# abowman6/CBET_RayTracing_3D

Measured on AMD Instinct MI355X. Metric: ray-steps/sec, OMEGA 60-beam 256^3 sweep, higher is better.
Workload: dtype f64

## Files before the change

### cbet_raytracing_3d_amd/csrc/cbet_trace_diag.h

```cpp
#ifndef CBET_TRACE_DIAG_H_
#define CBET_TRACE_DIAG_H_

#include "cbet_trace_common.h"

namespace cbet {

#ifdef CBET_DIAG_CLOCKS
#define CBET_IF_CLOCKS(...) __VA_ARGS__
#else
#define CBET_IF_CLOCKS(...)
#endif
#ifdef CBET_DIAG_FACES
#define CBET_IF_FACES(...) __VA_ARGS__
#else
#define CBET_IF_FACES(...)
#endif
#ifdef CBET_DIAG_CHAIN
#define CBET_IF_CHAIN(...) __VA_ARGS__
#else
#define CBET_IF_CHAIN(...)
#endif

struct WaveDiag {
    typedef unsigned long long u64;
    static constexpr bool kCountsWaveSteps = (0 CBET_IF_CLOCKS(+1) CBET_IF_FACES(+1) CBET_IF_CHAIN(+1)) != 0;
    CBET_IF_CLOCKS(u64 wait = 0, arm = 0, n_arm = 0, ret = 0, n_ret = 0, t_start, t_wait, t_arm, t_ret;)
    CBET_IF_FACES(unsigned near_steps = 0, near_axes = 0, arm_steps = 0;)
    CBET_IF_CHAIN(u64 chain = 0, t_chain = 0;)

    static __device__ __forceinline__ void stamp(u64 &t) { asm volatile("s_memtime %0" : "=&s"(t) : : "memory"); }
    static __device__ __forceinline__ void stamp_wait(u64 &t) { asm volatile("s_memtime %0\n\ts_waitcnt lgkmcnt(0)" : "=&s"(t) : : "memory"); }
    static __device__ __forceinline__ u64 since(u64 t0)
    {
        u64 t1;
        asm volatile("s_memtime %0\n\ts_waitcnt lgkmcnt(0)" : "=&s"(t1) : "s"(t0) : "memory");
        return t1 - t0;
    }

    __device__ __forceinline__ void begin() { CBET_IF_CLOCKS(stamp_wait(t_start);) }
    __device__ __forceinline__ void step_begin(int near)
    {
        (void)near;
        CBET_IF_FACES(near_steps += near != 0 ? 1 : 0; near_axes += __builtin_popcount((unsigned)near);)
    }
    __device__ __forceinline__ void wait_begin() { CBET_IF_CLOCKS(stamp(t_wait);) }
    __device__ __forceinline__ void wait_end()
    {
        CBET_IF_CLOCKS(wait += since(t_wait);)
        CBET_IF_CHAIN(stamp_wait(t_chain);)
    }
    __device__ __forceinline__ void chain_end() { CBET_IF_CHAIN(chain += since(t_chain);) }
    __device__ __forceinline__ void arm_begin()
    {
        CBET_IF_FACES(arm_steps += 1;)
        CBET_IF_CLOCKS(stamp(t_arm);)
    }
    __device__ __forceinline__ void arm_end() { CBET_IF_CLOCKS(arm += since(t_arm); n_arm += 1;) }
    __device__ __forceinline__ void retire_begin() { CBET_IF_CLOCKS(stamp(t_ret);) }
    __device__ __forceinline__ void retire_end() { CBET_IF_CLOCKS(ret += since(t_ret); n_ret += 1;) }
    __device__ __forceinline__ bool report(const TraceArgs &a, int lane, int tot_steps, int tot_rays, unsigned wave_steps)
    {
        auto put = [&](int slot, u64 v) { atomicAdd(&a.counters[slot], v); };
        if (kCountsWaveSteps && lane == 0) {
            CBET_IF_CLOCKS(u64 t_end; stamp_wait(t_end);)
            put(kCntSteps, (u64)tot_steps);
            put(kCntWaveSteps, (u64)wave_steps);
#if defined(CBET_DIAG_CLOCKS)
            put(kCntGlobalAtomics, wait);
            put(kCntEvictions, arm);
            put(kCntWaveStepsWide, n_arm);
            put(kCntSlabsRetired, t_end - t_start);
            put(kCntRays, ret);
            put(kCntWaveStepsMiss, n_ret);
#elif defined(CBET_DIAG_CHAIN)
            put(kCntRays, (u64)tot_rays);
            put(kCntGlobalAtomics, chain);
#elif defined(CBET_DIAG_FACES)
            put(kCntRays, (u64)tot_rays);
            put(kCntWaveStepsWide, (u64)near_steps);
            put(kCntWaveStepsMiss, (u64)near_axes);
            put(kCntSlabsRetired, (u64)arm_steps);
#endif
        }
        (void)tot_rays;
        return kCountsWaveSteps;
    }
};
#undef CBET_IF_CLOCKS
#undef CBET_IF_FACES
#undef CBET_IF_CHAIN

}

#endif
```

### cbet_raytracing_3d_amd/csrc/cbet_trace_window.hip

```cpp
#include <hip/hip_runtime.h>

#include <cstddef>
#include <type_traits>

#if defined(__HIP_DEVICE_COMPILE__) && !defined(__gfx950__)
#error "cbet_trace_window.hip is written for gfx950 (CDNA4) only"
#endif

#include "cbet_trace_common.h"
#include "cbet_trace_diag.h"

namespace cbet {
namespace {

#define CBET_BALLOT(cond) __builtin_amdgcn_ballot_w64(cond)
#define CBET_LANES(mask) __builtin_amdgcn_inverse_ballot_w64(mask)

template <int WX_, int WY_, int WZ_, bool PAD, bool XORSW = false>
struct Tile {
    static constexpr int WX = WX_, WY = WY_, WZ = WZ_;
    static constexpr int XM = WX - 1, YM = WY - 1, ZM = WZ - 1;
    static constexpr bool ROT = PAD && WZ == 16;
    static constexpr int YS = (PAD && !ROT) ? WZ + 1 : WZ;
    static constexpr int XS = (PAD && !ROT) ? WY * YS + 4 : WY * WZ;
    static constexpr bool XOR = ROT && XORSW;
    static __device__ __forceinline__ int zr(int tx, int ty, int tz)
    {
        return XOR ? (tz ^ ((tx & 3) << 2) ^ (ty << 1)) : (ROT ? ((tz + 7 * tx + 3 * ty) & ZM) : tz);
    }
    static_assert(!XOR || (WX == 8 && WY == 8 && WZ == 16), "the swizzle terms are written for the 8 x 8 x 16 box");
    static __device__ __forceinline__ int xterm(int tx) { return __mul24(tx, XS * 8 + 32) & ~0x80; }
    static __device__ __forceinline__ int yterm(int ty) { return __mul24(ty, YS * 8 + 16); }
    static constexpr int N = WX * XS;
    static constexpr int SX = WX - 2, SY = WY - 2, SZ = WZ - 2;
    static constexpr bool BRICK = WZ == 16 && WY == 8;
    static constexpr int DT = WX * WY * WZ;
    static __device__ __forceinline__ int slot_d(int tx, int ty, int tz) { return (tx * WY + ty) * WZ + tz; }
};

struct Origin {
    int x, y, z;
};

template <int M>
__device__ __forceinline__ int abs_in(int o, int r) { return o + ((r - o) & M); }

template <int C>
struct Corner {
    static constexpr int index = C;
    template <class V> static __device__ __forceinline__ V x(V v0, V v1) { return (C & 1) ? v1 : v0; }
    template <class V> static __device__ __forceinline__ V z(V v0, V v1) { return (C & 2) ? v1 : v0; }
    template <class V> static __device__ __forceinline__ V y(V v0, V v1) { return (C & 4) ? v1 : v0; }
};
template <class F>
__device__ __forceinline__ void each_corner(F f)
{
    f(Corner<0>{}); f(Corner<1>{}); f(Corner<2>{}); f(Corner<3>{}); f(Corner<4>{}); f(Corner<5>{}); f(Corner<6>{}); f(Corner<7>{});
}

struct WaveCounters {
    int n_atomics = 0;
    int n_miss = 0;
    unsigned steps_miss = 0;
    unsigned slabs_bsteps = 0;
    int pend = 0;
    [[no_unique_address]] WaveDiag dg;
};

template <bool W32>
struct Grid {
    double *p;
};
template <bool W32>
__device__ __forceinline__ void grid_add(const TraceArgs &a, Grid<W32> g, int node, double v)
{
    if constexpr (W32) global_add(a, reinterpret_cast<double *>(reinterpret_cast<char *>(g.p) + ((unsigned)node * 8u)), v);
    else global_add(a, &g.p[node], v);
}
template <bool W32>
__device__ __forceinline__ void grid_add_far(const TraceArgs &a, Grid<W32> g, long index, double v) { global_add(a, &g.p[index], v); }

template <class G>
__device__ __forceinline__ void write_back(const TraceArgs &a, double *tile, int slot, G edep, int node, double v, WaveCounters &wc)
{
    wc.pend += (CBET_BALLOT(v != 0.0) != 0ull) ? 1 : 0;
    if (v != 0.0) {
        tile[slot] = 0.0;
        ++wc.n_atomics;
        grid_add(a, edep, node, v);
    }
}
template <class G>
__device__ __forceinline__ void write_back_far(const TraceArgs &a, double *tile, int slot, G edep, long index, double v, WaveCounters &wc)
{
    wc.pend += (CBET_BALLOT(v != 0.0) != 0ull) ? 1 : 0;
    if (v != 0.0) {
        grid_add_far(a, edep, index, v);
        tile[slot] = 0.0;
        ++wc.n_atomics;
    }
}

template <class F>
__device__ __forceinline__ void miss_add8(unsigned long long hbm_m, WaveCounters &wc, F add8)
{
    if (hbm_m != 0ull) {
        wc.pend += 8;
        if (CBET_LANES(hbm_m)) add8();
    }
}

template <class T, int AX, int COUNT, class G>
__device__ __forceinline__ void retire_planes(const TraceArgs &a, double *tile, const Origin &o, int coord, int step,
                                              int lane, G edep, int sXh, int sYh, WaveCounters &wc)
{
    constexpr int WO = AX == 0 ? T::WY : T::WX, OM = WO - 1;
    constexpr int IT = (WO * T::WZ + kWave - 1) / kWave;
    constexpr int RS = kWave / T::WZ;
    static_assert(IT == 1 || (IT == 2 && 2 * RS == WO), "a plane is one entry per lane, or two in the halves of the other axis");
    static_assert(!T::XOR || IT == 1 || (RS == 4 && T::YS == 16 && T::XS == 128), "the second entry's slot is written for the 8 x 8 x 16 box");
    constexpr int SLOT_X = AX == 0 ? (RS * T::YS) ^ ((2 * RS) & T::ZM) : RS * T::XS;
    const int r0 = lane / T::WZ, r1 = lane & T::ZM, k = abs_in<T::ZM>(o.z, r1);
    const int d0 = (r0 - (AX == 0 ? o.y : o.x)) & OM, dnode = ((d0 & RS) ? -RS : RS) * (AX == 0 ? sYh : sXh);
    const bool in_plane = !(WO * T::WZ < kWave) || lane < WO * T::WZ;
    double v[COUNT * IT];
    int slot[COUNT * IT], node[COUNT * IT];
#pragma unroll
    for (int pl = 0; pl < COUNT; ++pl) {
        const int c = coord + pl * step;
        const int fixed = c & (AX == 0 ? T::XM : T::YM);
#pragma unroll
        for (int e = 0; e < IT; ++e) {
            const int q = pl * IT + e, re = r0 + e * RS;
            if (e == 1 && T::XOR) {
                slot[q] = slot[q - 1] ^ SLOT_X;
                node[q] = node[q - 1] + dnode;
            } else if (AX == 0) {
                slot[q] = fixed * T::XS + re * T::YS + T::zr(fixed, re, r1);
                node[q] = c * sXh + __mul24(abs_in<T::YM>(o.y, re), sYh) + k;
            } else {
                slot[q] = re * T::XS + fixed * T::YS + T::zr(re, fixed, r1);
                node[q] = __mul24(abs_in<T::XM>(o.x, re), sXh) + c * sYh + k;
            }
            const bool ok = in_plane && CBET_AUDIT(a, (unsigned)slot[q] < (unsigned)T::N);
            v[q] = ok ? tile[slot[q]] : 0.0;
        }
    }
#pragma unroll
    for (int q = 0; q < COUNT * IT; ++q) write_back(a, tile, slot[q], edep, node[q], v[q], wc);
}

template <class T, int AX, int NC, class G>
__device__ __forceinline__ void retire_plane(const TraceArgs &a, double *tile, const Origin &o, int coord, int lane,
                                             G edep, int sXh, int sYh, WaveCounters &wc, int coff, long gstride)
{
    constexpr int WO = AX == 0 ? T::WY : T::WX;
    constexpr int IT = (WO * T::WZ + kWave - 1) / kWave;
    const int fixed = coord & (AX == 0 ? T::XM : T::YM);
#pragma unroll
    for (int e = 0; e < IT; ++e) {
        const int idx = e * kWave + lane;
        const bool in_plane = !(WO * T::WZ < kWave) || idx < WO * T::WZ;
        const int r0 = idx / T::WZ, r1 = idx & T::ZM;
        int slot, node, slot_d;
        const int k = abs_in<T::ZM>(o.z, r1);
        if (AX == 0) {
            slot = fixed * T::XS + r0 * T::YS + T::zr(fixed, r0, r1);
            slot_d = T::slot_d(fixed, r0, r1);
            node = coord * sXh + __mul24(abs_in<T::YM>(o.y, r0), sYh) + k;
        } else {
            slot = r0 * T::XS + fixed * T::YS + T::zr(r0, fixed, r1);
            slot_d = T::slot_d(r0, fixed, r1);
            node = __mul24(abs_in<T::XM>(o.x, r0), sXh) + coord * sYh + k;
        }
        const bool ok = in_plane && CBET_AUDIT(a, (unsigned)slot < (unsigned)T::N);
        const double v = ok ? tile[slot] : 0.0;
        if (NC > 1) {
#pragma unroll
            for (int q = 1; q < NC; ++q) {
                const int sq = coff + (q - 1) * T::DT + slot_d;
                write_back_far(a, tile, sq, edep, q * gstride + node, ok ? tile[sq] : 0.0, wc);
            }
        }
        write_back(a, tile, slot, edep, node, v, wc);
    }
}

template <class T, int NC, class G>
__device__ __forceinline__ void retire_zplane(const TraceArgs &a, double *tile, const Origin &o, int coord, int lane,
                                              G edep, int sXh, int sYh, WaveCounters &wc, int coff, long gstride)
{
    static_assert(T::WX * T::WY <= kWave, "one z-plane entry per lane");
    const int r0 = lane / T::WY, r1 = lane & T::YM, fixed = coord & T::ZM;
    const int slot = r0 * T::XS + r1 * T::YS + T::zr(r0, r1, fixed);
    const int node = __mul24(abs_in<T::XM>(o.x, r0), sXh) + __mul24(abs_in<T::YM>(o.y, r1), sYh) + coord;
    const bool ok = (!(T::WX * T::WY < kWave) || lane < T::WX * T::WY) && CBET_AUDIT(a, (unsigned)slot < (unsigned)T::N);
    const double v = ok ? tile[slot] : 0.0;
    if (NC > 1) {
        const int slot_d = T::slot_d(r0, r1, fixed);
#pragma unroll
        for (int q = 1; q < NC; ++q) {
            const int sq = coff + (q - 1) * T::DT + slot_d;
            write_back_far(a, tile, sq, edep, q * gstride + node, ok ? tile[sq] : 0.0, wc);
        }
    }
    write_back(a, tile, slot, edep, node, v, wc);
}

template <class T, class G>
__device__ __forceinline__ void retire_zbrick(const TraceArgs &a, double *tile, const Origin &o, int zb, int lane,
                                              G edep, int sXh, int sYh, WaveCounters &wc)
{
    static_assert(T::WY == 8 && T::WZ == 16, "a brick is 8 rows of 8 planes per tile x index");
    const int ty = lane >> 3, kz = lane & 7;
    const int tz = (zb + kz) & T::ZM;
    const int base_node = __mul24(abs_in<T::YM>(o.y, ty), sYh) + zb + kz;
    constexpr int ROUND = 4;
#pragma unroll
    for (int t0 = 0; t0 < T::WX; t0 += ROUND) {
        double v[ROUND];
        int slot[ROUND];
#pragma unroll
        for (int q = 0; q < ROUND; ++q) {
            slot[q] = (t0 + q) * T::XS + ty * T::YS + T::zr(t0 + q, ty, tz);
            v[q] = CBET_AUDIT(a, (unsigned)slot[q] < (unsigned)T::N) ? tile[slot[q]] : 0.0;
        }
#pragma unroll
        for (int q = 0; q < ROUND; ++q) write_back(a, tile, slot[q], edep, abs_in<T::XM>(o.x, t0 + q) * sXh + base_node, v[q], wc);
    }
}

template <class T, int NC, class G>
__device__ __forceinline__ void flush_box(const TraceArgs &a, double *tile, const Origin &o, int lane, G edep,
                                          int sXh, int sYh, WaveCounters &wc, int coff, long gstride)
{
    for (int t = 0; t < T::WX; ++t)
        retire_plane<T, 0, NC>(a, tile, o, o.x + t, lane, edep, sXh, sYh, wc, coff, gstride);
}

__device__ __forceinline__ int follow_plane_axis(int r, unsigned long long mm, int S)
{
    const unsigned long long edge = __builtin_amdgcn_ballot_w64((unsigned)(r - 1) >= (unsigned)(S - 1)) & mm;
    if (edge == 0ull) return 0;
    const unsigned long long hi = __builtin_amdgcn_ballot_w64(r >= S) & edge;
    const bool at_hi = hi != 0ull, at_lo = hi != edge;
    if (at_hi == at_lo) return 0;
    if (at_hi) {
        if ((__builtin_amdgcn_ballot_w64(r <= 1) & mm) != 0ull) return (__builtin_amdgcn_ballot_w64(r > S) & mm) != 0ull ? 1 : 0;
        return (S >= 6 && (__builtin_amdgcn_ballot_w64(r <= 2) & mm) == 0ull) ? 2 : 1;
    }
    if ((__builtin_amdgcn_ballot_w64(r >= S - 1) & mm) != 0ull) return (__builtin_amdgcn_ballot_w64(r < 0) & mm) != 0ull ? -1 : 0;
    return (S >= 6 && (__builtin_amdgcn_ballot_w64(r >= S - 2) & mm) == 0ull) ? -2 : -1;
}

__device__ __forceinline__ int follow_brick_axis(int r, unsigned long long mm)
{
    if ((__builtin_amdgcn_ballot_w64((unsigned)r > 14u) & mm) == 0ull) return 0;
    const bool below = (__builtin_amdgcn_ballot_w64(r < 0) & mm) != 0ull, above = (__builtin_amdgcn_ballot_w64(r > 14) & mm) != 0ull;
    const bool needs_lo = (__builtin_amdgcn_ballot_w64(r <= 7) & mm) != 0ull, needs_hi = (__builtin_amdgcn_ballot_w64(r >= 7) & mm) != 0ull;
    return (below && !needs_hi) ? -1 : ((above && !needs_lo) ? 1 : 0);
}

template <class T, int NC, class G>
__device__ __forceinline__ bool follow_box(const TraceArgs &a, double *tile, Origin &o, unsigned long long mm, int lx,
                                           int ly, int lz, int lane, G edep, int sXh, int sYh, WaveCounters &wc,
                                           int coff, long gstride)
{
    auto leave = [&](auto axis, int d, int lo, int hi) {
        constexpr int AX = decltype(axis)::value;
        const int first = d < 0 ? hi : lo, step = d < 0 ? -1 : 1, n = d < 0 ? -d : d;
        if constexpr (NC == 1) {
            if (n == 2) retire_planes<T, AX, 2>(a, tile, o, first, step, lane, edep, sXh, sYh, wc);
            else retire_planes<T, AX, 1>(a, tile, o, first, step, lane, edep, sXh, sYh, wc);
        } else {
            for (int q = 0; q < n; ++q) retire_plane<T, AX, NC>(a, tile, o, first + q * step, lane, edep, sXh, sYh, wc, coff, gstride);
        }
    };
    const int dx = follow_plane_axis(lx - o.x, mm, T::SX);
    const int dy = follow_plane_axis(ly - o.y, mm, T::SY);
    if (dx != 0) { wc.dg.retire_begin(); leave(std::integral_constant<int, 0>{}, dx, o.x, o.x + T::WX - 1); wc.dg.retire_end(); }
    o.x += dx;
    if (dy != 0) { wc.dg.retire_begin(); leave(std::integral_constant<int, 1>{}, dy, o.y, o.y + T::WY - 1); wc.dg.retire_end(); }
    o.y += dy;
    int dz;
    if constexpr (T::BRICK) {
        dz = 8 * follow_brick_axis(lz - o.z, mm);
        if (dz != 0) { wc.dg.retire_begin(); retire_zbrick<T>(a, tile, o, dz < 0 ? o.z + 8 : o.z, lane, edep, sXh, sYh, wc); wc.dg.retire_end(); }
    } else {
        dz = follow_plane_axis(lz - o.z, mm, T::SZ);
        if (dz != 0)
            retire_zplane<T, NC>(a, tile, o, dz < 0 ? o.z + T::WZ - 1 : o.z, lane, edep, sXh, sYh, wc, coff, gstride);
        for (int q = 1; q < (dz < 0 ? -dz : dz); ++q)
            retire_zplane<T, NC>(a, tile, o, dz < 0 ? o.z + T::WZ - 1 - q : o.z + q, lane, edep, sXh, sYh, wc, coff, gstride);
    }
    o.z += dz;
    const bool moved = (dx | dy | dz) != 0;
    wc.slabs_bsteps += moved ? (1u << 16) : 0u;
    return moved;
}

template <class T>
__device__ __forceinline__ bool holds(const Origin &o, int lx, int ly, int lz)
{
    return (unsigned)(lx - o.x) <= (unsigned)T::SX && (unsigned)(ly - o.y) <= (unsigned)T::SY &&
           (unsigned)(lz - o.z) <= (unsigned)T::SZ;
}

template <class T>
__device__ __forceinline__ int box_near_axes(const Origin &o, int nx, int ny, int nz)
{
    const int lo = kRelocateDeep + 1;
    const unsigned tx = (unsigned)((o.x - lo) | (nx - 3 - T::SX - o.x)), ty = (unsigned)((o.y - lo) | (ny - 3 - T::SY - o.y)),
                   tz = (unsigned)((o.z - lo) | (nz - 3 - T::SZ - o.z));
    return (int)((tx >> 31) | ((ty >> 31) << 1) | ((tz >> 31) << 2));
}

typedef double dbl2 __attribute__((ext_vector_type(2)));

template <bool WIDE>
__device__ __forceinline__ void record_issue(const StepRecord *base, unsigned cell, dbl2 &kxy, dbl2 &kzk)
{
    if constexpr (WIDE) {
        const char *p = reinterpret_cast<const char *>(base) + ((unsigned long long)cell << 5);
        asm volatile("global_load_dwordx4 %0, %2, off\n\tglobal_load_dwordx4 %1, %2, off offset:16\n\t; CBET_RECORD_ISSUE %0 %1"
                     : "=&v"(kxy), "=&v"(kzk)
                     : "v"(p)
                     : "memory");
    } else {
        const unsigned off = cell << 5;
        asm volatile("s_nop 4\n\tglobal_load_dwordx4 %0, %2, %3\n\tglobal_load_dwordx4 %1, %2, %3 offset:16\n\t; CBET_RECORD_ISSUE %0 %1"
                     : "=&v"(kxy), "=&v"(kzk)
                     : "v"(off), "s"(base)
                     : "memory");
    }
}

__device__ __forceinline__ void record_wait(dbl2 &kxy, dbl2 &kzk, int pend)
{
    asm volatile("; CBET_RECORD_WAIT %0 %1\n\t"
                 "s_cmp_eq_u32 %2, 0\n\t"
                 "s_cbranch_scc1 .Lrw_0_%=\n\t"
                 "s_cmp_ge_u32 %2, 8\n\t"
                 "s_cbranch_scc1 .Lrw_8_%=\n\t"
                 "s_cmp_ge_u32 %2, 4\n\t"
                 "s_cbranch_scc1 .Lrw_4_%=\n\t"
                 "s_cmp_ge_u32 %2, 2\n\t"
                 "s_cbranch_scc1 .Lrw_2_%=\n\t"
                 "s_waitcnt vmcnt(1)\n\t"
                 "s_branch .Lrw_end_%=\n"
                 ".Lrw_2_%=:\n\t"
                 "s_waitcnt vmcnt(2)\n\t"
                 "s_branch .Lrw_end_%=\n"
                 ".Lrw_4_%=:\n\t"
                 "s_waitcnt vmcnt(4)\n\t"
                 "s_branch .Lrw_end_%=\n"
                 ".Lrw_8_%=:\n\t"
                 "s_waitcnt vmcnt(8)\n\t"
                 "s_branch .Lrw_end_%=\n"
                 ".Lrw_0_%=:\n\t"
                 "s_waitcnt vmcnt(0)\n"
                 ".Lrw_end_%=:"
                 : "+v"(kxy), "+v"(kzk)
                 : "s"(pend)
                 : "memory", "scc");
}

__device__ __forceinline__ void record_wait_all(dbl2 &kxy, dbl2 &kzk)
{
    asm volatile("; CBET_RECORD_WAIT %0 %1\n\ts_waitcnt vmcnt(0)" : "+v"(kxy), "+v"(kzk) : : "memory");
}

__device__ __forceinline__ void exit_planes_load(dbl2 &bx, dbl2 &by, dbl2 &bz)
{
    const void *args = (const void *)__builtin_amdgcn_kernarg_segment_ptr();
    asm volatile("s_load_dwordx4 %0, %3, %4\n\ts_load_dwordx4 %1, %3, %5\n\ts_load_dwordx4 %2, %3, %6\n\ts_waitcnt lgkmcnt(0)"
                 : "=&s"(bx), "=&s"(by), "=&s"(bz)
                 : "s"(args), "i"(offsetof(TraceArgs, exit_planes)), "i"(offsetof(TraceArgs, exit_planes) + 16),
                   "i"(offsetof(TraceArgs, exit_planes) + 32));
}

__device__ __forceinline__ int add3(int a, int b, int c)
{
    int r;
    asm("v_add3_u32 %0, %1, %2, %3" : "=v"(r) : "v"(a), "v"(b), "v"(c));
    return r;
}

__device__ __forceinline__ int xad1(int f, int c)
{
    int r;
    asm("v_xad_u32 %0, %1, 1, %2" : "=v"(r) : "v"(f), "v"(c));
    return r;
}

__device__ __forceinline__ double max_abs3(double a, double b, double c)
{
    double r;
    asm("v_max_f64 %0, |%1|, |%2|" : "=v"(r) : "v"(a), "v"(b));
    asm("v_max_f64 %0, %1, |%2|" : "=v"(r) : "v"(r), "v"(c));
    return r;
}

__device__ __forceinline__ void commit(int &var, int value)
{
    asm volatile("s_mov_b32 %0, %1" : "+s"(var) : "s"(__builtin_amdgcn_readfirstlane(value)));
}
__device__ __forceinline__ void commit(unsigned long long &var, unsigned long long value)
{
    asm volatile("s_mov_b64 %0, %1" : "+s"(var) : "s"(value));
}
__device__ __forceinline__ void commit_v(int &var, int value) { asm volatile("v_mov_b32 %0, %1" : "+v"(var) : "v"(value)); }

__device__ __forceinline__ void cell_step(int &c, unsigned long long up, unsigned long long dn)
{
    asm("s_nop 1\n\tv_addc_co_u32_e64 %0, vcc, 0, %0, %1\n\tv_subbrev_co_u32_e64 %0, vcc, 0, %0, %2" : "+v"(c) : "s"(up), "s"(dn) : "vcc");
}
__device__ __forceinline__ void cell_step3(int &ci, int &cj, int &ck, unsigned long long upx, unsigned long long dnx,
                                           unsigned long long upy, unsigned long long dny, unsigned long long upz,
                                           unsigned long long dnz)
{
    asm("s_nop 1\n\t"
        "v_addc_co_u32_e64 %0, vcc, 0, %0, %3\n\tv_addc_co_u32_e64 %1, vcc, 0, %1, %5\n\tv_addc_co_u32_e64 %2, vcc, 0, %2, %7\n\t"
        "v_subbrev_co_u32_e64 %0, vcc, 0, %0, %4\n\tv_subbrev_co_u32_e64 %1, vcc, 0, %1, %6\n\tv_subbrev_co_u32_e64 %2, vcc, 0, %2, %8"
        : "+v"(ci), "+v"(cj), "+v"(ck)
        : "s"(upx), "s"(dnx), "s"(upy), "s"(dny), "s"(upz), "s"(dnz)
        : "vcc");
}

__device__ __forceinline__ int mad24(int a, int b, int c)
{
    int r;
    asm("s_nop 1\n\tv_mad_i32_i24 %0, %1, %2, %3" : "=v"(r) : "v"(a), "s"(b), "v"(c));
    return r;
}


#ifdef CBET_DEBUG_BOUNDS
constexpr bool kAudited = true;
#else
constexpr bool kAudited = false;
#endif
constexpr double kNearTol = 0.5001;
constexpr double kFarJump = 1.4998;

template <int WZ, bool GENERIC, int CBET, bool STATS>
__global__ void __launch_bounds__(kWave, (CBET == 4) ? 1 : 4) k_trace_window(const TraceArgs a)
{
    using T = Tile<8, 8, WZ, true, CBET == 0>;
    using TB = Tile<4, 8, 8, false>;
    constexpr bool IDX64 = GENERIC;
    constexpr int NC = (CBET == 4) ? 4 : 1;
    constexpr bool ACC = (CBET == 0);
    constexpr bool PIPE = ACC;
    constexpr int NSLOT = T::N + TB::N;
    constexpr int NLDS = NSLOT + (NC - 1) * T::DT;
    __shared__ double s_val[NLDS];
    const int lane = threadIdx.x;

    int beam, patch;
    if (!work_item(a, blockIdx.x, beam, patch)) return;
    const Grid<!IDX64> edep{a.edep + (long)(beam - a.grid_beam0) * a.grid_stride};
    const bool absorb = GENERIC ? (a.absorption == 1) : true;

    Ray s = {};
    int li;
    const bool launched = launch_lane(a, beam, patch, lane, s, li);
    unsigned long long live = __ballot(launched);
    if (live == 0ull) return;
    const int tot_rays = __popcll(live);

    const int nx = a.nx, ny = a.ny, nz = a.nz;
    const int sYh = a.sYh, sXh = a.sXh;
    unsigned cell = launched ? (unsigned)((s.ci * ny + s.cj) * nz + s.ck) : 0u;
    double fcx = (double)s.ci, fcy = (double)s.cj, fcz = (double)s.ck;
    int tot_steps = 0;
    WaveCounters wc;

    double *const tileA = s_val, *const tileB = s_val + T::N;
    Origin oA{0, 0, 0}, oB{0, 0, 0};
    unsigned long long hbm = 0ull;
    int b_active = 0;
    {
        const int src = ((live >> 27) & 1ull) ? 27 : (__ffsll((long long)live) - 1);
        for (int z = lane; z < NLDS; z += kWave) s_val[z] = 0.0;
        oA.x = __builtin_amdgcn_readlane(s.ci, src) + 1 - T::WX / 2;
        oA.y = __builtin_amdgcn_readlane(s.cj, src) + 1 - T::WY / 2;
        oA.z = __builtin_amdgcn_readlane(s.ck, src) + 1 - 4;
        if (T::BRICK) oA.z &= ~7;
        __syncthreads();
    }
    int near = 7;
    wc.dg.begin();

    dbl2 rec_kxy, rec_kzk;
    const StepRecord *rec_base = a.steprec;
    asm volatile("" : "+s"(rec_base));
    double dt = a.dt;
    auto gather_record = [&]() {
        unsigned c = CBET_LANES(live) ? cell : 0u;
        asm("" : "+v"(c));
#ifdef CBET_DEBUG_BOUNDS
        if (!(c < a.audit_nodes)) { audit_fail(a); c = 0u; }
#endif
        record_issue<IDX64>(rec_base, c, rec_kxy, rec_kzk);
        wc.pend = 0;
    };
    auto await_record = [&]() {
        wc.dg.wait_begin();
        if (CBET == 0 && !kAudited) record_wait(rec_kxy, rec_kzk, wc.pend);
        else record_wait_all(rec_kxy, rec_kzk);
        wc.dg.wait_end();
    };
    gather_record();
    await_record();
    const double *const gk = CBET && a.gain ? a.gain + (long)(beam - a.grid_beam0) * a.hsize : nullptr;
    double gained = 0.0;

    const bool flx = (lane & 1) != 0, fly = (lane & 2) != 0, flz = (lane & 8) != 0;
    const int pfx = flx ? 1 : 0, pfy = fly ? 1 : 0, pfz = flz ? 1 : 0;

    double q0 = 0.0, q1 = 0.0, q2 = 0.0, q3 = 0.0;

    int slow = 7;
    double Fx0 = 0, Fx1 = 0, Fy0 = 0, Fy1 = 0, Fz0 = 0, Fz1 = 0;
    int X0 = 0, X1 = 0, Y0 = 0, Y1 = 0, Z0 = 0, Z1 = 0;
    double inc = 0.0;
    int tile_off = 0;
    unsigned long long miss_m = 0ull;
    int own_slot = 0, own_node = 0;
    auto lds_add8 = [&](const double *w) {
        auto add = [&](int byte, double v) {
            if (CBET_AUDIT(a, (unsigned)byte < (unsigned)NSLOT * 8u))
                __hip_atomic_fetch_add(static_cast<double *>(__builtin_assume_aligned(reinterpret_cast<char *>(s_val) + byte, 8)),
                                       v, __ATOMIC_RELAXED, __HIP_MEMORY_SCOPE_WORKGROUP);
        };
        if constexpr (T::XOR) {
            int ax0, ax1, by0, by1, cz0, cz1;
            if (b_active == 0) {
                ax0 = T::xterm(X0 & T::XM); ax1 = T::xterm(X1 & T::XM);
                by0 = T::yterm(Y0 & T::YM); by1 = T::yterm(Y1 & T::YM);
                cz0 = (Z0 & T::ZM) << 3; cz1 = (Z1 & T::ZM) << 3;
            } else {
                const bool toB = tile_off != 0;
                const int xm = toB ? TB::XM : T::XM, zm = toB ? TB::ZM : T::ZM;
                const int xmul = toB ? TB::XS * 8 : T::XS * 8 + 32, ymul = toB ? TB::YS * 8 : T::YS * 8 + 16;
                const int keep = toB ? ~0 : ~0x80, off8 = tile_off * 8;
                static_assert(TB::YM == T::YM, "one y mask for both boxes");
                ax0 = (__mul24(X0 & xm, xmul) & keep) | off8; ax1 = (__mul24(X1 & xm, xmul) & keep) | off8;
                by0 = __mul24(Y0 & T::YM, ymul); by1 = __mul24(Y1 & T::YM, ymul);
                cz0 = (Z0 & zm) << 3; cz1 = (Z1 & zm) << 3;
            }
            auto at = [](int ax, int by, int cz) { return (int)__builtin_amdgcn_bitop3_b32(ax, by, cz, 0x96); };
            each_corner([=](auto c) { add(at(c.x(ax0, ax1), c.y(by0, by1), c.z(cz0, cz1)), w[c.index]); });
        } else {
            auto add8 = [&](int xm, int ym, int zm, int xs, int ys, int off, int rot) {
                const int xa = X0 & xm, xb = X1 & xm, ya = Y0 & ym, yb = Y1 & ym;
                const int x0 = __mul24(xa, xs * 8) + off * 8, x1 = __mul24(xb, xs * 8) + off * 8;
                const int y0 = __mul24(ya, ys * 8), y1 = __mul24(yb, ys * 8);
                const int ra = 7 * xa * rot, rb = 7 * xb * rot, sa = 3 * ya * rot, sb = 3 * yb * rot;
                auto zb = [&](int z, int r) { return ((z + r) & zm) * 8; };
                if constexpr (T::ROT) {
                    const int xy00 = x0 | y0, xy10 = x1 | y0, xy01 = x0 | y1, xy11 = x1 | y1, zm8 = zm * 8;
                    auto at = [&](int xy, int z, int r) { return (((z + r) * 8) & zm8) | xy; };
                    each_corner([&](auto c) {
                        add(at(c.y(c.x(xy00, xy10), c.x(xy01, xy11)), c.z(Z0, Z1), c.x(ra, rb) + c.y(sa, sb)), w[c.index]);
                    });
                } else {
                    each_corner([&](auto c) {
                        add(add3(c.x(x0, x1), c.y(y0, y1), zb(c.z(Z0, Z1), c.x(ra, rb) + c.y(sa, sb))), w[c.index]);
                    });
                }
            };
            if (b_active == 0) {
                add8(T::XM, T::YM, T::ZM, T::XS, T::YS, 0, T::ROT ? 1 : 0);
            } else {
                const bool toB = tile_off != 0;
                add8(toB ? TB::XM : T::XM, toB ? TB::YM : T::YM, toB ? TB::ZM : T::ZM, toB ? TB::XS : T::XS,
                     toB ? TB::YS : T::YS, tile_off, (T::ROT && !toB) ? 1 : 0);
            }
        }
    };
    auto hbm_add8 = [&](const double *w) {
        const int nX0 = __mul24(X0, sXh), nX1 = __mul24(X1, sXh), nY0 = __mul24(Y0, sYh), nY1 = __mul24(Y1, sYh);
        each_corner([&](auto c) { grid_add(a, edep, c.x(nX0, nX1) + c.y(nY0, nY1) + c.z(Z0, Z1), w[c.index]); });
        wc.n_atomics += 8;
    };

    auto deposit_step = [&](unsigned long long lds_m, unsigned long long hbm_m) {
        const double zi0 = Fz0 * inc, zi1 = Fz1 * inc;
        const double zy00 = zi0 * Fy0, zy10 = zi1 * Fy0, zy01 = zi0 * Fy1, zy11 = zi1 * Fy1;
        double wgt[8];
        wgt[0] = zy00 * Fx0;
        wgt[1] = zy00 * Fx1;
        wgt[2] = zy10 * Fx0;
        wgt[3] = zy10 * Fx1;
        wgt[4] = zy01 * Fx0;
        wgt[5] = zy01 * Fx1;
        wgt[6] = zy11 * Fx0;
        wgt[7] = zy11 * Fx1;
        if (CBET_LANES(lds_m)) lds_add8(wgt);
        miss_add8(hbm_m, wc, [&]() {
            hbm_add8(wgt);
            ++wc.n_miss;
        });
        if (CBET == 4) {
            const bool inbox = CBET_LANES(lds_m);
            if (inbox && tile_off == 0) {
                if (CBET_AUDIT(a, (unsigned)(own_slot + 2 * T::DT) < (unsigned)NLDS)) {
                    __hip_atomic_fetch_add(&s_val[own_slot], q1, __ATOMIC_RELAXED, __HIP_MEMORY_SCOPE_WORKGROUP);
                    __hip_atomic_fetch_add(&s_val[own_slot + T::DT], q2, __ATOMIC_RELAXED, __HIP_MEMORY_SCOPE_WORKGROUP);
                    __hip_atomic_fetch_add(&s_val[own_slot + 2 * T::DT], q3, __ATOMIC_RELAXED, __HIP_MEMORY_SCOPE_WORKGROUP);
                }
            } else if (inbox || CBET_LANES(hbm_m)) {
                grid_add_far(a, edep, a.comp_stride + own_node, q1);
                grid_add_far(a, edep, 2 * a.comp_stride + own_node, q2);
                grid_add_far(a, edep, 3 * a.comp_stride + own_node, q3);
                wc.n_atomics += 3;
            }
        }
    };

    double S[8] = {0, 0, 0, 0, 0, 0, 0, 0};
    unsigned long long restart_m = 0ull;
    bool p_odd = true;
    auto accumulate = [&]() {
        const double zi0 = Fz0 * inc, zi1 = Fz1 * inc;
        const double zy00 = zi0 * Fy0, zy10 = zi1 * Fy0, zy01 = zi0 * Fy1, zy11 = zi1 * Fy1;
        const double k = CBET_LANES(restart_m) ? 0.0 : 1.0;
        auto add = [&](double &sum, double w) { asm("v_fma_f64 %0, %0, %1, %2" : "+v"(sum) : "v"(k), "v"(w)); };
        add(S[0], zy00 * Fx0);
        add(S[1], zy00 * Fx1);
        add(S[2], zy10 * Fx0);
        add(S[3], zy10 * Fx1);
        add(S[4], zy01 * Fx0);
        add(S[5], zy01 * Fx1);
        add(S[6], zy11 * Fx0);
        add(S[7], zy11 * Fx1);
    };
    auto flush_sums = [&](unsigned long long lds_m, unsigned long long hbm_m) {
        if (CBET_LANES(lds_m)) lds_add8(S);
        miss_add8(hbm_m, wc, [&]() { hbm_add8(S); });
    };

    auto step_tail = [&](int &tt) {
    asm volatile("" : "+v"(Fx0), "+v"(Fx1), "+v"(Fy0), "+v"(Fy1), "+v"(Fz0), "+v"(Fz1));
    await_record();
    if (absorb) {
        inc = rec_kzk.y * s.uray;
        s.uray -= inc;
    } else {
        inc = s.uray;
    }
    if (CBET >= 2) inc = q0;
    if constexpr (ACC && !PIPE) accumulate();
    unsigned long long died = CBET_BALLOT(s.uray <= s.ustop);
    const int faces = slow | near;
    if (faces != 0) {
        dbl2 bx, by, bz;
        exit_planes_load(bx, by, bz);
        if (faces & 1) died |= CBET_BALLOT(s.px < bx.x) | CBET_BALLOT(s.px > bx.y);
        if (faces & 2) died |= CBET_BALLOT(s.py < by.x) | CBET_BALLOT(s.py > by.y);
        if (faces & 4) died |= CBET_BALLOT(s.pz < bz.x) | CBET_BALLOT(s.pz > bz.y);
    }
    died &= live;
    if (died != 0ull) {
        asm volatile("");
        commit(tot_steps, tot_steps + __popcll(died) * (tt + 1));
        if constexpr (PIPE) {
            accumulate();
            asm volatile("v_mov_b64 %0, 0" : "+v"(inc));
            commit(restart_m, 0ull);
        }
        if constexpr (ACC) flush_sums(died & ~miss_m, died & miss_m);
        else deposit_step(died & ~miss_m, died & miss_m);
        commit(live, live & ~died);
        commit(hbm, hbm & live);
        commit(miss_m, miss_m & live);
        if (live == 0ull) commit(tt, a.nt - 1);
    }
    __builtin_amdgcn_wave_barrier();
    };

    for (int tt = 0; tt < a.nt; ++tt) {
        if constexpr (STATS || WaveDiag::kCountsWaveSteps) wc.steps_miss += 1u << 16;
        wc.dg.step_begin(near);
        s.vx -= rec_kxy.x;
        s.vy -= rec_kxy.y;
        s.vz -= rec_kzk.x;
        asm volatile("" : "+s"(dt));
        s.px += s.vx * dt;
        s.py += s.vy * dt;
        s.pz += s.vz * dt;
        const double fx = (s.px - a.xmin) * a.inv_dx;
        const double fy = (s.py - a.ymin) * a.inv_dy;
        const double fz = (s.pz - a.zmin) * a.inv_dz;
        const double g0x = fx - fcx, g0y = fy - fcy, g0z = fz - fcz;
        const unsigned long long upx = CBET_BALLOT(g0x >= kNearTol), dnx = CBET_BALLOT(g0x < kNearTol - 1.0),
                                 upy = CBET_BALLOT(g0y >= kNearTol), dny = CBET_BALLOT(g0y < kNearTol - 1.0),
                                 upz = CBET_BALLOT(g0z >= kNearTol), dnz = CBET_BALLOT(g0z < kNearTol - 1.0);
        slow = ((CBET_BALLOT(!(max_abs3(g0x, g0y, g0z) < kFarJump)) & live) != 0ull) ? 7 : near;
        if (slow == 0) {
            cell_step3(s.ci, s.cj, s.ck, upx, dnx, upy, dny, upz, dnz);
        } else {
            if (slow & 1) s.ci = relocate_closed(s.ci, fx, nx);
            else cell_step(s.ci, upx, dnx);
            if (slow & 2) s.cj = relocate_closed(s.cj, fy, ny);
            else cell_step(s.cj, upy, dny);
            if (slow & 4) s.ck = relocate_closed(s.ck, fz, nz);
            else cell_step(s.ck, upz, dnz);
        }
        const unsigned new_cell = (unsigned)mad24(mad24(s.ci, ny, s.cj), nz, s.ck);
        unsigned long long moved_m = 0ull;
        if constexpr (ACC) moved_m = CBET_BALLOT(new_cell != cell);
        cell = new_cell;
        gather_record();
        wc.dg.chain_end();
        asm volatile("" : "+v"(s.ci), "+v"(s.cj), "+v"(s.ck), "+v"(inc));
        fcx = (double)s.ci;
        fcy = (double)s.cj;
        fcz = (double)s.ck;
        if constexpr (!ACC) deposit_step(live & ~miss_m, miss_m);
        if constexpr (PIPE) accumulate();
        const double ox = (fx - fcx) - 0.5, oy = (fy - fcy) - 0.5, oz = (fz - fcz) - 0.5;
        const bool ngx = ox < 0, ngy = oy < 0, ngz = oz < 0;
        const bool all_negative = (live & ~(CBET_BALLOT(ngx) & CBET_BALLOT(ngy) & CBET_BALLOT(ngz))) == 0ull;
        if constexpr (ACC) {
            const unsigned long long fl_m = (all_negative && !p_odd) ? (live & moved_m) : live;
            if (fl_m != 0ull) {
                if (miss_m == 0ull) flush_sums(fl_m, 0ull);
                else flush_sums(fl_m & ~miss_m, fl_m & miss_m);
            }
            restart_m = fl_m;
            p_odd = !all_negative;
        }
        factor_pair(ox, pfx, Fx0, Fx1);
        factor_pair(oy, pfy, Fy0, Fy1);
        factor_pair(oz, pfz, Fz0, Fz1);
        int rx, ry, rz;
        if (all_negative) {
            rx = s.ci - oA.x;
            ry = s.cj - oA.y;
            rz = s.ck - oA.z;
            asm("" : "+v"(rx), "+v"(ry), "+v"(rz));
            X0 = xad1(pfx, s.ci); X1 = s.ci + pfx;
            Y0 = xad1(pfy, s.cj); Y1 = s.cj + pfy;
            Z0 = xad1(pfz, s.ck); Z1 = s.ck + pfz;
        } else {
            const int lx = s.ci + 1 - (ngx ? 1 : 0);
            const int ly = s.cj + 1 - (ngy ? 1 : 0);
            const int lz = s.ck + 1 - (ngz ? 1 : 0);
            rx = lx - oA.x;
            ry = ly - oA.y;
            rz = lz - oA.z;
            const bool hx = ngx != flx, hy = ngy != fly, hz = ngz != flz;
            X0 = lx + (hx ? 1 : 0); X1 = lx + (hx ? 0 : 1);
            Y0 = ly + (hy ? 1 : 0); Y1 = ly + (hy ? 0 : 1);
            Z0 = lz + (hz ? 1 : 0); Z1 = lz + (hz ? 0 : 1);
        }
        if (CBET && CBET_LANES(live)) {
            double ds = 0.0;
            if (gk || CBET >= 2) ds = sqrt_speed(__builtin_fma(s.vz, s.vz, __builtin_fma(s.vy, s.vy, s.vx * s.vx))) * a.dt;
            double u_eff = s.uray;
            if (gk) {
                const double x = gain_exponent<IDX64>(a, gk, X0, X1, Y0, Y1, Z0, Z1, Fx0, Fx1, Fy0, Fy1, Fz0, Fz1, sXh, sYh, ds);
                const double phi = gain_phi(x, (CBET_BALLOT(!(fabs(x) < kPhiSmallBelow)) & live) == 0ull);
                const double dg = s.uray * (x * phi);
                u_eff = s.uray * phi;
                gained += dg;
                s.uray = s.uray + dg;
            }
            if (CBET == 2) q0 = u_eff * ds;
            if (CBET == 4) {
                q0 = u_eff * ds;
                q1 = u_eff * (s.vx * a.dt);
                q2 = u_eff * (s.vy * a.dt);
                q3 = u_eff * (s.vz * a.dt);
                const int hi = s.ci + 1, hj = s.cj + 1, hk = s.ck + 1;
                own_slot = T::slot_d(hi & T::XM, hj & T::YM, hk & T::ZM) + NSLOT;
                own_node = __mul24(hi, sXh) + __mul24(hj, sYh) + hk;
            }
        }
        const unsigned long long memA = live & ~hbm;
        unsigned long long out_core = memA & ~(CBET_BALLOT((unsigned)rx <= (unsigned)T::SX) & CBET_BALLOT((unsigned)ry <= (unsigned)T::SY) &
                                               CBET_BALLOT((unsigned)rz <= (unsigned)T::SZ));
        if (b_active != 0) {
            asm volatile("");
            if constexpr (STATS) wc.slabs_bsteps += 1u;
            const int abx = oA.x - oB.x, aby = oA.y - oB.y, abz = oA.z - oB.z;
            out_core |= hbm & ~(CBET_BALLOT((unsigned)(rx + abx) <= (unsigned)TB::SX) &
                                CBET_BALLOT((unsigned)(ry + aby) <= (unsigned)TB::SY) &
                                CBET_BALLOT((unsigned)(rz + abz) <= (unsigned)TB::SZ));
            tile_off = CBET_LANES(hbm) ? T::N : 0;
        }
        out_core |= miss_m;
        if (out_core != 0ull) {
            wc.dg.arm_begin();
            const bool alive = CBET_LANES(live);
            int lx = rx + oA.x, ly = ry + oA.y, lz = rz + oA.z;
            asm volatile("" : "+v"(lx), "+v"(ly), "+v"(lz));
            Origin nA = oA, nB = oB;
            unsigned long long n_hbm = hbm, n_miss = 0ull;
            int n_bact = b_active, n_near, n_toff = tile_off;
            follow_box<T, NC>(a, tileA, nA, memA, lx, ly, lz, lane, edep, sXh, sYh, wc, NSLOT, a.comp_stride);
            const unsigned long long lost_mask =
                memA & ~(CBET_BALLOT((unsigned)(lx - nA.x) <= (unsigned)T::SX) & CBET_BALLOT((unsigned)(ly - nA.y) <= (unsigned)T::SY) &
                         CBET_BALLOT((unsigned)(lz - nA.z) <= (unsigned)T::SZ));
            if (lost_mask == 0ull && n_bact == 0) {
                n_near = box_near_axes<T>(nA, nx, ny, nz);
            } else {
                bool homeB = CBET_LANES(hbm);
                const bool inA = alive && holds<T>(nA, lx, ly, lz);
                const bool lost = alive && !homeB && !inA;
                if (n_bact != 0) {
                    follow_box<TB, 1>(a, tileB, nB, hbm, lx, ly, lz, lane, edep, sXh, sYh, wc, 0, 0);
                } else if (lost_mask != 0ull) {
                    const int src = __ffsll((long long)lost_mask) - 1;
                    const int sx = __builtin_amdgcn_readlane(lx, src), sy = __builtin_amdgcn_readlane(ly, src),
                              sz = __builtin_amdgcn_readlane(lz, src);
                    nB.x = sx - (TB::WX / 2 - 1);
                    nB.y = sy - (TB::WY / 2 - 1);
                    nB.z = sz - TB::SZ / 2;
                    n_bact = 1;
                }
                const bool inB = alive && holds<TB>(nB, lx, ly, lz);
                homeB = homeB || (lost && inB);
                if (alive && homeB && !inB && inA) homeB = false;
                n_hbm = CBET_BALLOT(alive && homeB);
                if (n_hbm == 0ull) {
                    __builtin_amdgcn_wave_barrier();
                    flush_box<TB, 1>(a, tileB, nB, lane, edep, sXh, sYh, wc, 0, 0);
                    n_bact = 0;
                }
                __builtin_amdgcn_wave_barrier();
                const bool useB = alive && homeB && inB;
                n_toff = useB ? T::N : 0;
                n_miss = live & ~CBET_BALLOT(useB || (alive && !homeB && inA));
                if constexpr (STATS) {
                    if (n_miss != 0ull) wc.steps_miss += 1u;
                    if (ACC && CBET_LANES(n_miss)) ++wc.n_miss;
                }
                n_near = n_miss != 0ull ? 7 : (box_near_axes<T>(nA, nx, ny, nz) | (n_bact == 0 ? 0 : box_near_axes<TB>(nB, nx, ny, nz)));
            }
            commit(oA.x, nA.x); commit(oA.y, nA.y); commit(oA.z, nA.z);
            commit(oB.x, nB.x); commit(oB.y, nB.y); commit(oB.z, nB.z);
            commit(hbm, n_hbm); commit(miss_m, n_miss);
            commit(b_active, n_bact); commit(near, n_near);
            commit_v(tile_off, n_toff);
            wc.pend = __builtin_amdgcn_readfirstlane(wc.pend);
            wc.dg.arm_end();
        } else if (near != 0) {
            commit(near, box_near_axes<T>(oA, nx, ny, nz) | (b_active == 0 ? 0 : box_near_axes<TB>(oB, nx, ny, nz)));
        }
        step_tail(tt);
    }
    tot_steps += __popcll(live) * a.nt;

    if constexpr (PIPE) accumulate();
    if constexpr (ACC) flush_sums(live & ~miss_m, live & miss_m);
    else deposit_step(live & ~miss_m, live & miss_m);
    __syncthreads();
    flush_box<T, NC>(a, tileA, oA, lane, edep, sXh, sYh, wc, NSLOT, a.comp_stride);
    if (b_active != 0) flush_box<TB, 1>(a, tileB, oB, lane, edep, sXh, sYh, wc, 0, 0);

    if (CBET && a.beam_gain) {
        double t = gained;
#pragma unroll
        for (int off = 32; off > 0; off >>= 1) t += __shfl_xor(t, off, kWave);
        if (lane == 0 && t != 0.0) atomicAdd(&a.beam_gain[beam], t);
    }
    if (wc.dg.report(a, lane, tot_steps, tot_rays, wc.steps_miss >> 16)) return;
    if constexpr (STATS) {
        const int tot_at = wave_sum(wc.n_atomics), tot_miss = wave_sum(wc.n_miss);
        if (lane == 0) {
            atomicAdd(&a.counters[kCntGlobalAtomics], (unsigned long long)tot_at);
            atomicAdd(&a.counters[kCntEvictions], (unsigned long long)tot_miss);
            atomicAdd(&a.counters[kCntWaveSteps], (unsigned long long)(wc.steps_miss >> 16));
            atomicAdd(&a.counters[kCntWaveStepsMiss], (unsigned long long)(wc.steps_miss & 0xFFFFu));
            atomicAdd(&a.counters[kCntWaveStepsWide], (unsigned long long)(wc.slabs_bsteps & 0xFFFFu));
            atomicAdd(&a.counters[kCntSlabsRetired], (unsigned long long)(wc.slabs_bsteps >> 16));
        }
    }
    if (lane == 0) {
        atomicAdd(&a.counters[kCntSteps], (unsigned long long)tot_steps);
        atomicAdd(&a.counters[kCntRays], (unsigned long long)tot_rays);
    }
}

}

hipError_t launch_trace_window(const TraceArgs &a, bool force_idx64, hipStream_t stream)
{
    const long waves = a.item_count;
    if (waves <= 0) return hipSuccess;
    const dim3 grid((unsigned)waves), block(kWave);
    const unsigned long long grid_bytes = 8ull * (unsigned long long)a.sXh * (unsigned long long)(a.nx + 2);
    const bool generic = force_idx64 || (a.gain && 8ull * (unsigned long long)a.hsize >= (1ull << 32)) || a.absorption != 1 ||
                         grid_bytes >= (1ull << 32) ||
                         sizeof(StepRecord) * (unsigned long long)a.nx * a.ny * a.nz > (1ull << 32);
    auto go = [&](auto wz, auto cbet) {
        constexpr int WZ = decltype(wz)::value, CB = decltype(cbet)::value;
        if (a.stats) {
            if (generic) hipLaunchKernelGGL((k_trace_window<WZ, true, CB, true>), grid, block, 0, stream, a);
            else hipLaunchKernelGGL((k_trace_window<WZ, false, CB, true>), grid, block, 0, stream, a);
        } else {
            if (generic) hipLaunchKernelGGL((k_trace_window<WZ, true, CB, false>), grid, block, 0, stream, a);
            else hipLaunchKernelGGL((k_trace_window<WZ, false, CB, false>), grid, block, 0, stream, a);
        }
    };
    using std::integral_constant;
    if (a.quantity == 1) go(integral_constant<int, 8>{}, integral_constant<int, 4>{});
    else if (a.quantity == 2) go(integral_constant<int, 16>{}, integral_constant<int, 2>{});
    else if (a.gain || a.beam_gain) go(integral_constant<int, 16>{}, integral_constant<int, 1>{});
    else go(integral_constant<int, 16>{}, integral_constant<int, 0>{});
    return hipGetLastError();
}

}
```

Before: 174.0 billion.

## Narrow near-axis flags for miss lanes and refine record wait counts

When some lanes miss both boxes, the near-boundary flag was forced to all three axes. It now checks per axis, through a wave ballot, whether any missing lane's cell is near the grid edge, so fewer axes take the boundary-handling path on later steps. The record wait ladder is extended so it can wait for exactly vmcnt(N) for every N up to 16, rather than rounding down to a power of two, which avoids draining more loads than needed. A compile-time-gated diagnostic mode that counts arm and miss causes is also added; it compiles out by default.

```diff
diff --git a/cbet_raytracing_3d_amd/csrc/cbet_trace_diag.h b/cbet_raytracing_3d_amd/csrc/cbet_trace_diag.h
--- a/cbet_raytracing_3d_amd/csrc/cbet_trace_diag.h
+++ b/cbet_raytracing_3d_amd/csrc/cbet_trace_diag.h
@@ -20,13 +20,25 @@
 #else
 #define CBET_IF_CHAIN(...)
 #endif
+#ifdef CBET_DIAG_CAUSES
+#define CBET_IF_CAUSES(...) __VA_ARGS__
+#else
+#define CBET_IF_CAUSES(...)
+#endif
 
 struct WaveDiag {
     typedef unsigned long long u64;
-    static constexpr bool kCountsWaveSteps = (0 CBET_IF_CLOCKS(+1) CBET_IF_FACES(+1) CBET_IF_CHAIN(+1)) != 0;
+    static constexpr bool kCountsWaveSteps = (0 CBET_IF_CLOCKS(+1) CBET_IF_FACES(+1) CBET_IF_CHAIN(+1) CBET_IF_CAUSES(+1)) != 0;
     CBET_IF_CLOCKS(u64 wait = 0, arm = 0, n_arm = 0, ret = 0, n_ret = 0, t_start, t_wait, t_arm, t_ret;)
     CBET_IF_FACES(unsigned near_steps = 0, near_axes = 0, arm_steps = 0;)
     CBET_IF_CHAIN(u64 chain = 0, t_chain = 0;)
+    enum { kEvArmMissOnly = 32, kEvArmOther = 33, kEvNear7Miss = 34, kEvNear7Other = 35, kEvMissFlushes = 36, kEvMissFlushLanes = 37 };
+    CBET_IF_CAUSES(unsigned bins = 0; int lane_id = 0;)
+    __device__ __forceinline__ void count(int bin, unsigned by = 1u)
+    {
+        (void)bin; (void)by;
+        CBET_IF_CAUSES(bins += lane_id == bin ? by : 0u;)
+    }
 
     static __device__ __forceinline__ void stamp(u64 &t) { asm volatile("s_memtime %0" : "=&s"(t) : : "memory"); }
     static __device__ __forceinline__ void stamp_wait(u64 &t) { asm volatile("s_memtime %0\n\ts_waitcnt lgkmcnt(0)" : "=&s"(t) : : "memory"); }
@@ -37,11 +49,31 @@
         return t1 - t0;
     }
 
-    __device__ __forceinline__ void begin() { CBET_IF_CLOCKS(stamp_wait(t_start);) }
-    __device__ __forceinline__ void step_begin(int near)
+    __device__ __forceinline__ void begin()
     {
-        (void)near;
+        CBET_IF_CLOCKS(stamp_wait(t_start);)
+        CBET_IF_CAUSES(lane_id = (int)__builtin_amdgcn_mbcnt_hi(~0u, __builtin_amdgcn_mbcnt_lo(~0u, 0u));)
+    }
+    __device__ __forceinline__ void step_begin(int near, u64 miss_m)
+    {
+        (void)near; (void)miss_m;
         CBET_IF_FACES(near_steps += near != 0 ? 1 : 0; near_axes += __builtin_popcount((unsigned)near);)
+        CBET_IF_CAUSES(if (near == 7) count(miss_m != 0ull ? kEvNear7Miss : kEvNear7Other);)
+    }
+    __device__ __forceinline__ void wait_pend(int pend)
+    {
+        (void)pend;
+        CBET_IF_CAUSES(count(pend > 16 ? 17 : pend);)
+    }
+    __device__ __forceinline__ void miss_flush(u64 hbm_m)
+    {
+        (void)hbm_m;
+        CBET_IF_CAUSES(count(kEvMissFlushes); count(kEvMissFlushLanes, (unsigned)__builtin_popcountll(hbm_m));)
+    }
+    __device__ __forceinline__ void arm_cause(u64 out_core, u64 miss_m)
+    {
+        (void)out_core; (void)miss_m;
+        CBET_IF_CAUSES(if ((out_core | miss_m) != 0ull) count((out_core & ~miss_m) == 0ull ? kEvArmMissOnly : kEvArmOther);)
     }
     __device__ __forceinline__ void wait_begin() { CBET_IF_CLOCKS(stamp(t_wait);) }
     __device__ __forceinline__ void wait_end()
@@ -61,6 +93,15 @@
     __device__ __forceinline__ bool report(const TraceArgs &a, int lane, int tot_steps, int tot_rays, unsigned wave_steps)
     {
         auto put = [&](int slot, u64 v) { atomicAdd(&a.counters[slot], v); };
+#if defined(CBET_DIAG_CAUSES)
+        {
+            const int c = lane < 18 ? lane : ((lane >= 32 && lane < 38) ? lane - 14 : -1);
+            if (c >= 0 && c / 12 == (CBET_DIAG_CAUSES) && bins != 0u) {
+                const int k = c % 12, s = k >> 1;
+                put(s < 3 ? s + 1 : s + 2, (u64)bins << (32 * (k & 1)));
+            }
+        }
+#endif
         if (kCountsWaveSteps && lane == 0) {
             CBET_IF_CLOCKS(u64 t_end; stamp_wait(t_end);)
             put(kCntSteps, (u64)tot_steps);
@@ -75,6 +116,7 @@
 #elif defined(CBET_DIAG_CHAIN)
             put(kCntRays, (u64)tot_rays);
             put(kCntGlobalAtomics, chain);
+#elif defined(CBET_DIAG_CAUSES)
 #elif defined(CBET_DIAG_FACES)
             put(kCntRays, (u64)tot_rays);
             put(kCntWaveStepsWide, (u64)near_steps);
@@ -89,6 +131,7 @@
 #undef CBET_IF_CLOCKS
 #undef CBET_IF_FACES
 #undef CBET_IF_CHAIN
+#undef CBET_IF_CAUSES
 
 }
 
diff --git a/cbet_raytracing_3d_amd/csrc/cbet_trace_window.hip b/cbet_raytracing_3d_amd/csrc/cbet_trace_window.hip
--- a/cbet_raytracing_3d_amd/csrc/cbet_trace_window.hip
+++ b/cbet_raytracing_3d_amd/csrc/cbet_trace_window.hip
@@ -106,6 +106,7 @@
 {
     if (hbm_m != 0ull) {
         wc.pend += 8;
+        wc.dg.miss_flush(hbm_m);
         if (CBET_LANES(hbm_m)) add8();
     }
 }
@@ -315,6 +316,15 @@
     return (int)((tx >> 31) | ((ty >> 31) << 1) | ((tz >> 31) << 2));
 }
 
+__device__ __forceinline__ int cell_near_axes(unsigned long long m, int ci, int cj, int ck, int nx, int ny, int nz)
+{
+    auto some_outside = [&](int c, int n) {
+        const int deep_cells = n - 2 - kRelocateDeep;
+        return (CBET_BALLOT((unsigned)(c - kRelocateDeep) >= (unsigned)(deep_cells > 0 ? deep_cells : 0)) & m) != 0ull;
+    };
+    return (some_outside(ci, nx) ? 1 : 0) | (some_outside(cj, ny) ? 2 : 0) | (some_outside(ck, nz) ? 4 : 0);
+}
+
 typedef double dbl2 __attribute__((ext_vector_type(2)));
 
 template <bool WIDE>
@@ -340,22 +350,82 @@
     asm volatile("; CBET_RECORD_WAIT %0 %1\n\t"
                  "s_cmp_eq_u32 %2, 0\n\t"
                  "s_cbranch_scc1 .Lrw_0_%=\n\t"
+                 "s_cmp_ge_u32 %2, 9\n\t"
+                 "s_cbranch_scc1 .Lrw_ge9_%=\n\t"
+                 "s_cmp_ge_u32 %2, 5\n\t"
+                 "s_cbranch_scc1 .Lrw_ge5_%=\n\t"
+                 "s_cmp_ge_u32 %2, 3\n\t"
+                 "s_cbranch_scc1 .Lrw_ge3_%=\n\t"
+                 "s_cmp_ge_u32 %2, 2\n\t"
+                 "s_cbranch_scc1 .Lrw_ge2_%=\n\t"
+                 "s_waitcnt vmcnt(1)\n\t"
+                 "s_branch .Lrw_end_%=\n"
+                 ".Lrw_ge2_%=:\n\t"
+                 "s_waitcnt vmcnt(2)\n\t"
+                 "s_branch .Lrw_end_%=\n"
+                 ".Lrw_ge3_%=:\n\t"
+                 "s_cmp_ge_u32 %2, 4\n\t"
+                 "s_cbranch_scc1 .Lrw_ge4_%=\n\t"
+                 "s_waitcnt vmcnt(3)\n\t"
+                 "s_branch .Lrw_end_%=\n"
+                 ".Lrw_ge4_%=:\n\t"
+                 "s_waitcnt vmcnt(4)\n\t"
+                 "s_branch .Lrw_end_%=\n"
+                 ".Lrw_ge5_%=:\n\t"
+                 "s_cmp_ge_u32 %2, 7\n\t"
+                 "s_cbranch_scc1 .Lrw_ge7_%=\n\t"
+                 "s_cmp_ge_u32 %2, 6\n\t"
+                 "s_cbranch_scc1 .Lrw_ge6_%=\n\t"
+                 "s_waitcnt vmcnt(5)\n\t"
+                 "s_branch .Lrw_end_%=\n"
+                 ".Lrw_ge6_%=:\n\t"
+                 "s_waitcnt vmcnt(6)\n\t"
+                 "s_branch .Lrw_end_%=\n"
+                 ".Lrw_ge7_%=:\n\t"
                  "s_cmp_ge_u32 %2, 8\n\t"
-                 "s_cbranch_scc1 .Lrw_8_%=\n\t"
-                 "s_cmp_ge_u32 %2, 4\n\t"
-                 "s_cbranch_scc1 .Lrw_4_%=\n\t"
-                 "s_cmp_ge_u32 %2, 2\n\t"
-                 "s_cbranch_scc1 .Lrw_2_%=\n\t"
-                 "s_waitcnt vmcnt(1)\n\t"
-                 "s_branch .Lrw_end_%=\n"
-                 ".Lrw_2_%=:\n\t"
-                 "s_waitcnt vmcnt(2)\n\t"
-                 "s_branch .Lrw_end_%=\n"
-                 ".Lrw_4_%=:\n\t"
-                 "s_waitcnt vmcnt(4)\n\t"
-                 "s_branch .Lrw_end_%=\n"
-                 ".Lrw_8_%=:\n\t"
+                 "s_cbranch_scc1 .Lrw_ge8_%=\n\t"
+                 "s_waitcnt vmcnt(7)\n\t"
+                 "s_branch .Lrw_end_%=\n"
+                 ".Lrw_ge8_%=:\n\t"
                  "s_waitcnt vmcnt(8)\n\t"
+                 "s_branch .Lrw_end_%=\n"
+                 ".Lrw_ge9_%=:\n\t"
+                 "s_cmp_ge_u32 %2, 13\n\t"
+                 "s_cbranch_scc1 .Lrw_ge13_%=\n\t"
+                 "s_cmp_ge_u32 %2, 11\n\t"
+                 "s_cbranch_scc1 .Lrw_ge11_%=\n\t"
+                 "s_cmp_ge_u32 %2, 10\n\t"
+                 "s_cbranch_scc1 .Lrw_ge10_%=\n\t"
+                 "s_waitcnt vmcnt(9)\n\t"
+                 "s_branch .Lrw_end_%=\n"
+                 ".Lrw_ge10_%=:\n\t"
+                 "s_waitcnt vmcnt(10)\n\t"
+                 "s_branch .Lrw_end_%=\n"
+                 ".Lrw_ge11_%=:\n\t"
+                 "s_cmp_ge_u32 %2, 12\n\t"
+                 "s_cbranch_scc1 .Lrw_ge12_%=\n\t"
+                 "s_waitcnt vmcnt(11)\n\t"
+                 "s_branch .Lrw_end_%=\n"
+                 ".Lrw_ge12_%=:\n\t"
+                 "s_waitcnt vmcnt(12)\n\t"
+                 "s_branch .Lrw_end_%=\n"
+                 ".Lrw_ge13_%=:\n\t"
+                 "s_cmp_ge_u32 %2, 15\n\t"
+                 "s_cbranch_scc1 .Lrw_ge15_%=\n\t"
+                 "s_cmp_ge_u32 %2, 14\n\t"
+                 "s_cbranch_scc1 .Lrw_ge14_%=\n\t"
+                 "s_waitcnt vmcnt(13)\n\t"
+                 "s_branch .Lrw_end_%=\n"
+                 ".Lrw_ge14_%=:\n\t"
+                 "s_waitcnt vmcnt(14)\n\t"
+                 "s_branch .Lrw_end_%=\n"
+                 ".Lrw_ge15_%=:\n\t"
+                 "s_cmp_ge_u32 %2, 16\n\t"
+                 "s_cbranch_scc1 .Lrw_ge16_%=\n\t"
+                 "s_waitcnt vmcnt(15)\n\t"
+                 "s_branch .Lrw_end_%=\n"
+                 ".Lrw_ge16_%=:\n\t"
+                 "s_waitcnt vmcnt(16)\n\t"
                  "s_branch .Lrw_end_%=\n"
                  ".Lrw_0_%=:\n\t"
                  "s_waitcnt vmcnt(0)\n"
@@ -644,6 +714,7 @@
 
     auto step_tail = [&](int &tt) {
     asm volatile("" : "+v"(Fx0), "+v"(Fx1), "+v"(Fy0), "+v"(Fy1), "+v"(Fz0), "+v"(Fz1));
+    wc.dg.wait_pend(wc.pend);
     await_record();
     if (absorb) {
         inc = rec_kzk.y * s.uray;
@@ -683,7 +754,7 @@
 
     for (int tt = 0; tt < a.nt; ++tt) {
         if constexpr (STATS || WaveDiag::kCountsWaveSteps) wc.steps_miss += 1u << 16;
-        wc.dg.step_begin(near);
+        wc.dg.step_begin(near, miss_m);
         s.vx -= rec_kxy.x;
         s.vy -= rec_kxy.y;
         s.vz -= rec_kzk.x;
@@ -792,6 +863,7 @@
                                 CBET_BALLOT((unsigned)(rz + abz) <= (unsigned)TB::SZ));
             tile_off = CBET_LANES(hbm) ? T::N : 0;
         }
+        wc.dg.arm_cause(out_core, miss_m);
         out_core |= miss_m;
         if (out_core != 0ull) {
             wc.dg.arm_begin();
@@ -839,7 +911,8 @@
                     if (n_miss != 0ull) wc.steps_miss += 1u;
                     if (ACC && CBET_LANES(n_miss)) ++wc.n_miss;
                 }
-                n_near = n_miss != 0ull ? 7 : (box_near_axes<T>(nA, nx, ny, nz) | (n_bact == 0 ? 0 : box_near_axes<TB>(nB, nx, ny, nz)));
+                n_near = box_near_axes<T>(nA, nx, ny, nz) | (n_bact == 0 ? 0 : box_near_axes<TB>(nB, nx, ny, nz));
+                if (n_miss != 0ull) n_near |= cell_near_axes(n_miss, s.ci, s.cj, s.ck, nx, ny, nz);
             }
             commit(oA.x, nA.x); commit(oA.y, nA.y); commit(oA.z, nA.z);
             commit(oB.x, nB.x); commit(oB.y, nB.y); commit(oB.z, nB.z);
```

Measured after the change: 175.5 billion, median of 6. No clear change (+0.8%).
